# sair-lab/AirSLAM

Measured on AMD Instinct MI355X. Metric: stereo detect+match pairs/sec (2x PLNet @512x512 internal: points + lines, junctions on the left + LightGlue match), higher is better.
Workload: dtype fp16

## Files before the change

### airslam_amd/csrc/kernels_lgblockf.hip

```cpp
#include "common.h"
#include "kernels.h"
#ifdef LF_TIMING
__device__ unsigned long long lf_dbg[32];
#define LF_T(i) { const long long now_ = wall_clock64(); if (L.wave == 0 && L.lane == 0) atomicAdd(&lf_dbg[L.tb + i], (unsigned long long)(now_ - tp_)); tp_ = now_; }
extern "C" void airfe_dbg_lf(unsigned long long* out, int reset) {
  if (reset) { unsigned long long z[32] = {}; (void)hipMemcpyToSymbol(HIP_SYMBOL(lf_dbg), z, sizeof(z)); }
  else (void)hipMemcpyFromSymbol(out, HIP_SYMBOL(lf_dbg), 32 * sizeof(unsigned long long));
}
#else
#define LF_T(i)
#endif
#ifdef LF_TIMING2
__device__ unsigned long long lf2_dbg[16];
extern "C" void airfe_dbg_lf2(unsigned long long* out, int reset) {
  if (reset) { unsigned long long z[16] = {}; (void)hipMemcpyToSymbol(HIP_SYMBOL(lf2_dbg), z, sizeof(z)); }
  else (void)hipMemcpyFromSymbol(out, HIP_SYMBOL(lf2_dbg), 16 * sizeof(unsigned long long));
}
#define LF2_NOW(v) { __builtin_amdgcn_sched_barrier(0); v = __builtin_readcyclecounter(); __builtin_amdgcn_sched_barrier(0); }
#endif

namespace airfe {

constexpr int LF_R0 = 0, LF_R1 = 65536, LF_ST = 131072;
constexpr int LF_LDS = LF_ST + 8 * 128 * 8;

#ifndef LF_FRAG
#define LF_FRAG 1
#endif
constexpr int LF_SS = LF_FRAG ? 2048 : SLAB_BYTES;
constexpr int lf_ts(int K) { return LF_FRAG ? (K / 64) * 2048 : 2048; }
constexpr int LF_TS256 = lf_ts(256), LF_TS512 = lf_ts(512);
__device__ __forceinline__ size_t lf_woff(int K, int cb, int t0) {
  return LF_FRAG ? (size_t)(cb * 4 + t0) * (K / 64) * 2048 : (size_t)cb * (K / 64) * SLAB_BYTES + (size_t)t0 * 2048;
}

__device__ __forceinline__ void lf_glds16(const void* gsrc, unsigned lds_off) {
  unsigned keep;
  asm volatile("s_mov_b32 %0, m0\n\ts_mov_b32 m0, %2\n\ts_nop 0\n\tglobal_load_lds_dwordx4 %1, off\n\ts_mov_b32 m0, %0"
               : "=&s"(keep)
               : "v"(gsrc), "s"(lds_off)
               : "memory");
}

#ifndef LF_GELU_ERFC
__device__ __forceinline__ f32x2 lf_gelu2(f32x2 y) {
  const f32x2 t = {__builtin_amdgcn_fmed3f(y.x, -4.5f, 4.5f), __builtin_amdgcn_fmed3f(y.y, -4.5f, 4.5f)};
  const f32x2 x = (t * t) * (2.0f / 20.25f) - 1.0f;
  f32x2 r = x * 0.0031705170404165983f - 0.009152771905064583f;
  r = r * x + 0.012448843568563461f;
  r = r * x - 0.016971856355667114f;
  r = r * x + 0.027542514726519585f;
  r = r * x - 0.040475402027368546f;
  r = r * x + 0.05482625961303711f;
  r = r * x - 0.07717858254909515f;
  r = r * x + 0.15690208971500397f;
  return y * (t * r + 0.5f);
}
__device__ __forceinline__ void lf_gelu2x4(f32x2 (&y)[4]) {
  f32x2 t[4], x[4], r[4];
#define LF_G4(expr) _Pragma("unroll") for (int k = 0; k < 4; ++k) { expr; } __builtin_amdgcn_sched_barrier(0);
  LF_G4((t[k] = f32x2{__builtin_amdgcn_fmed3f(y[k].x, -4.5f, 4.5f), __builtin_amdgcn_fmed3f(y[k].y, -4.5f, 4.5f)}))
  LF_G4(x[k] = t[k] * t[k])
  LF_G4(x[k] = x[k] * (2.0f / 20.25f) - 1.0f)
  LF_G4(r[k] = x[k] * 0.0031705170404165983f - 0.009152771905064583f)
  LF_G4(r[k] = r[k] * x[k] + 0.012448843568563461f)
  LF_G4(r[k] = r[k] * x[k] - 0.016971856355667114f)
  LF_G4(r[k] = r[k] * x[k] + 0.027542514726519585f)
  LF_G4(r[k] = r[k] * x[k] - 0.040475402027368546f)
  LF_G4(r[k] = r[k] * x[k] + 0.05482625961303711f)
  LF_G4(r[k] = r[k] * x[k] - 0.07717858254909515f)
  LF_G4(r[k] = r[k] * x[k] + 0.15690208971500397f)
  LF_G4(r[k] = t[k] * r[k] + 0.5f)
  LF_G4(y[k] = y[k] * r[k])
#undef LF_G4
}
#else
__device__ __forceinline__ f32x2 lf_gelu2(f32x2 y) {
  const f32x2 a = __builtin_elementwise_abs(y);
  f32x2 x = a * 0.70710678118654752f;
  x = __builtin_elementwise_min(x, f32x2{6.0f, 6.0f});
  const f32x2 u = x * (1.0f / 3.0f) - 1.0f;
  f32x2 r = u * 0.008399954997003078f - 0.02763195149600506f;
  r = r * u + 0.04838801920413971f;
  r = r * u - 0.08357185125350952f;
  r = r * u + 0.1567264348268509f;
  r = r * u - 0.28920042514801025f;
  r = r * u + 0.5534077286720276f;
  r = r * u - 1.3146467208862305f;
  r = r * u - 2.481963634490967f;
  const f32x2 p = (x * x) * -1.4426950408889634f + r;
  const f32x2 q = {__builtin_amdgcn_exp2f(p.x), __builtin_amdgcn_exp2f(p.y)};
  return __builtin_elementwise_max(y, f32x2{0.f, 0.f}) - (x * 0.70710678118654752f) * q;
}
__device__ __forceinline__ void lf_gelu2x4(f32x2 (&y)[4]) {
#pragma unroll
  for (int k = 0; k < 4; ++k) y[k] = lf_gelu2(y[k]);
}
#endif

__device__ __forceinline__ void lf_stage_rows(const uint16_t* src, int row0, int nmt, int region, int wave, int lane) {
  for (int i = 0; i < nmt; ++i) {
    const int inst = wave * nmt + i;
    const int r = inst * 2 + (lane >> 5), pp = lane & 31;
    lf_glds16(src + (size_t)(row0 + r) * 256 + ((pp ^ (r & 15)) << 3), (unsigned)(region + inst * 1024));
  }
}

template <class P>
__device__ __forceinline__ typename P::vec8 lf_ldg(const char* p) {
  return __builtin_bit_cast(typename P::vec8, *reinterpret_cast<const uint4*>(p));
}

template <class P, int NT, int TS>
__device__ __forceinline__ void lf_first(typename P::vec8 (&cur)[NT][2], const char* w0, const char* w1) {
#pragma unroll
  for (int t = 0; t < NT; ++t) {
    cur[t][0] = lf_ldg<P>(w0 + t * TS);
    cur[t][1] = lf_ldg<P>(w1 + t * TS);
  }
}

struct LfNoHook { __device__ __forceinline__ void operator()(int) const {} };

#ifndef LF_GELU_X4
#define LF_GELU_X4 1
#endif


template <class P, int NT, int NMT, int TS, int TSN, class Hook = LfNoHook, bool SWAP = false, bool TIMED = false>
__device__ __forceinline__ void lf_mma(f32x4 (&acc)[NT][NMT], typename P::vec8 (&cur)[NT][2], const char* w0, const char* w1, int nslab,
                                       const char* n0, const char* n1, const char* breg, int pitch, int l15, int g, Hook hook = Hook()) {
  const char* brow = breg + l15 * pitch;
  if constexpr (NMT <= 4) {
    typename P::vec8 ring[8][NT][2];
    auto fetch = [&](int k, typename P::vec8 (&dst)[NT][2]) {
      const char* p0 = k == nslab ? n0 : w0 + k * LF_SS;
      const char* p1 = k == nslab ? n1 : w1 + k * LF_SS;
      const int ts = k == nslab ? TSN : TS;
#pragma unroll
      for (int t = 0; t < NT; ++t) {
        dst[t][0] = lf_ldg<P>(p0 + t * ts);
        dst[t][1] = lf_ldg<P>(p1 + t * ts);
      }
    };
    constexpr int AHEAD = (NT == 4 ? 4 : 8) / (NMT > 2 ? 2 : 1);
#pragma unroll
    for (int d = 1; d <= AHEAD; ++d)
      if (d <= nslab) fetch(d, ring[d - 1]);
    __builtin_amdgcn_sched_barrier(0);
#pragma unroll
    for (int s = 0; s < 8; ++s) {
      if (s < nslab) {
        hook(s);
        __builtin_amdgcn_sched_barrier(0);
#pragma unroll
        for (int h = 0; h < 2; ++h) {
          const int boff = (((s * 8 + h * 4 + g) ^ l15) << 4);
          typename P::vec8 bf[NMT];
#pragma unroll
          for (int j = 0; j < NMT; ++j) bf[j] = lds_frag<P>(brow, boff + j * 16 * pitch);
#pragma unroll
          for (int t = 0; t < NT; ++t)
#pragma unroll
            for (int j = 0; j < NMT; ++j) {
              if constexpr (SWAP) acc[t][j] = P::mfma(bf[j], cur[t][h], acc[t][j]);
              else acc[t][j] = P::mfma(cur[t][h], bf[j], acc[t][j]);
            }
        }
#pragma unroll
        for (int t = 0; t < NT; ++t) {
          cur[t][0] = ring[s % AHEAD][t][0];
          cur[t][1] = ring[s % AHEAD][t][1];
        }
        if (s + 1 + AHEAD <= nslab) fetch(s + 1 + AHEAD, ring[s % AHEAD]);
        __builtin_amdgcn_sched_barrier(0);
      }
    }
    return;
  }
  typename P::vec8 nxt[NT][2];
#ifdef LF_NOLDS
  typename P::vec8 bf0[4];
#pragma unroll
  for (int j = 0; j < 4; ++j) bf0[j] = lds_frag<P>(brow, ((g ^ l15) << 4) + j * 16 * pitch);
#endif
#ifdef LF_TIMING2
  [[maybe_unused]] unsigned long long q0 = 0, q1 = 0, q2 = 0, q3 = 0, q4 = 0, q5 = 0, q6 = 0;
  [[maybe_unused]] unsigned long long a_pref = 0, a_vm = 0, a_rd = 0, a_lgkm = 0, a_mma = 0, a_mov = 0, a_trips = 0;
#endif
#pragma unroll 1
  for (int s = 0; s < nslab; ++s) {
#ifdef LF_TIMING2
    if constexpr (TIMED) LF2_NOW(q0)
#endif
    const bool last = s + 1 == nslab;
    const char* p0 = last ? n0 : w0 + (s + 1) * LF_SS;
    const char* p1 = last ? n1 : w1 + (s + 1) * LF_SS;
#ifdef LF_NOWEIGHTS
    if (true) {
      (void)p0; (void)p1;
#pragma unroll
      for (int t = 0; t < NT; ++t) {
        nxt[t][0] = cur[t][0];
        nxt[t][1] = cur[t][1];
      }
    } else
#endif
    if constexpr (TS == TSN) {
#pragma unroll
      for (int t = 0; t < NT; ++t) {
        nxt[t][0] = lf_ldg<P>(p0 + t * TS);
        nxt[t][1] = lf_ldg<P>(p1 + t * TS);
      }
    } else {
      const int ts = last ? TSN : TS;
#pragma unroll
      for (int t = 0; t < NT; ++t) {
        nxt[t][0] = lf_ldg<P>(p0 + t * ts);
        nxt[t][1] = lf_ldg<P>(p1 + t * ts);
      }
    }
    hook(s);
    __builtin_amdgcn_sched_barrier(0);
#ifdef LF_TIMING2
    if constexpr (TIMED) {
      LF2_NOW(q1)
      asm volatile("s_waitcnt vmcnt(%0)" ::"n"(2 * NT) : "memory");
      LF2_NOW(q2)
      a_pref += q1 - q0; a_vm += q2 - q1;
    }
#endif
#pragma unroll
    for (int h = 0; h < 2; ++h) {
      const int boff = (((s * 8 + h * 4 + g) ^ l15) << 4);
#pragma unroll
      for (int mb = 0; mb < NMT; mb += 4) {
#ifdef LF_TIMING2
        if constexpr (TIMED) LF2_NOW(q3)
#endif
        typename P::vec8 bf[4];
#ifdef LF_NOLDS
        (void)boff;
#pragma unroll
        for (int j = 0; j < 4; ++j) bf[j] = bf0[j];
#else
#pragma unroll
        for (int j = 0; j < 4; ++j)
          if (mb + j < NMT) bf[j] = lds_frag<P>(brow, boff + (mb + j) * 16 * pitch);
#endif
#ifdef LF_TIMING2
        if constexpr (TIMED) {
          LF2_NOW(q4)
          asm volatile("s_waitcnt lgkmcnt(0)" ::: "memory");
          LF2_NOW(q5)
        }
#endif
#pragma unroll
        for (int t = 0; t < NT; ++t)
#pragma unroll
          for (int j = 0; j < 4; ++j)
            if (mb + j < NMT) {
              if constexpr (SWAP) acc[t][mb + j] = P::mfma(bf[j], cur[t][h], acc[t][mb + j]);
              else acc[t][mb + j] = P::mfma(cur[t][h], bf[j], acc[t][mb + j]);
            }
#ifdef LF_TIMING2
        if constexpr (TIMED) {
          LF2_NOW(q6)
          a_rd += q4 - q3; a_lgkm += q5 - q4; a_mma += q6 - q5;
        }
#endif
      }
    }
#pragma unroll
    for (int t = 0; t < NT; ++t) {
      cur[t][0] = nxt[t][0];
      cur[t][1] = nxt[t][1];
    }
#ifdef LF_TIMING2
    if constexpr (TIMED) {
      LF2_NOW(q1)
      a_mov += q1 - q6; a_trips += 1;
    }
#endif
  }
#ifdef LF_TIMING2
  if constexpr (TIMED) {
    if ((threadIdx.x & 63) == 0) {
      atomicAdd(&lf2_dbg[0], a_pref); atomicAdd(&lf2_dbg[1], a_vm); atomicAdd(&lf2_dbg[2], a_rd); atomicAdd(&lf2_dbg[3], a_lgkm); atomicAdd(&lf2_dbg[4], a_mma);
      atomicAdd(&lf2_dbg[5], a_mov); atomicAdd(&lf2_dbg[6], a_trips); atomicAdd(&lf2_dbg[7], (unsigned long long)(2 * ((NMT + 3) / 4)) * a_trips);
      atomicAdd(&lf2_dbg[8], (unsigned long long)(2 * NT * NMT) * a_trips);
    }
  }
#endif
}

struct LfLane {
  int lane, wave, l15, g, wf, cb, tp, fo0, fo1;
#ifdef LF_TIMING
  int tb;
#endif
  const char *wob, *w1b, *w2b;
};

template <class P, int NMT, bool RELU, int FOLD, bool FOLDO>
__device__ __forceinline__ void lf_pass(const LgBlockFArgs& a, char* smem, const LfLane& L, int row0) {
  const int lane = L.lane, wave = L.wave, l15 = L.l15, g = L.g, wf = L.wf, cb = L.cb, tp = L.tp, fo0 = L.fo0, fo1 = L.fo1;
#ifdef LF_TIMING
  long long tp_ = wall_clock64();
  if (wave == 0 && lane == 0) atomicAdd(&lf_dbg[L.tb + 15], 1ull);
#endif
  typename P::vec8 c2[2][2], c4[4][2];
  [[maybe_unused]] f32x4 bo2[2];
  f32x4 b14[4];
  if constexpr (FOLDO) {
    lf_first<P, 4, LF_TS512>(c4, L.w1b + 4 * LF_SS + fo0, L.w1b + 4 * LF_SS + fo1);
  } else {
    lf_first<P, 2, LF_TS256>(c2, L.wob + fo0, L.wob + fo1);
#pragma unroll
    for (int u = 0; u < 2; ++u) bo2[u] = *reinterpret_cast<const f32x4*>(a.bo + cb * 64 + tp * 32 + g * 8 + u * 4);
  }
#pragma unroll
  for (int t = 0; t < 4; ++t) b14[t] = *reinterpret_cast<const f32x4*>(a.b1 + wf * 64 + (t >> 1) * 32 + g * 8 + (t & 1) * 4);
  asm volatile("s_waitcnt vmcnt(0)" ::: "memory");
  __syncthreads();
  LF_T(0)

  if constexpr (!FOLDO) {
    {
    f32x4 acc[2][NMT];
#pragma unroll
    for (int u = 0; u < 2; ++u)
#pragma unroll
      for (int m = 0; m < NMT; ++m) acc[u][m] = bo2[u];
    lf_mma<P, 2, NMT, LF_TS256, LF_TS256>(acc, c2, L.wob + fo0, L.wob + fo1, 4, L.wob + fo0, L.wob + fo1, smem + LF_R0, 512, l15, g);
    lf_first<P, 4, LF_TS512>(c4, L.w1b + 4 * LF_SS + fo0, L.w1b + 4 * LF_SS + fo1);
    const int piece = cb * 8 + tp * 4 + g;
#pragma unroll
    for (int m = 0; m < NMT; ++m) {
      float v[8];
#pragma unroll
      for (int e = 0; e < 4; ++e) {
        v[e] = acc[0][m][e];
        v[4 + e] = acc[1][m][e];
      }
      *reinterpret_cast<uint4*>(smem + LF_R1 + (m * 16 + l15) * 512 + ((piece ^ l15) << 4)) = pack8<P>(v);
    }
    }
    __syncthreads();
  }
  LF_T(1)

  f32x4 h[4][NMT];
#pragma unroll
  for (int t = 0; t < 4; ++t)
#pragma unroll
    for (int m = 0; m < NMT; ++m) h[t][m] = b14[t];
  if constexpr (FOLDO) {
    lf_mma<P, 4, NMT, LF_TS512, LF_TS512>(h, c4, L.w1b + 4 * LF_SS + fo0, L.w1b + 4 * LF_SS + fo1, 4, L.w1b + fo0, L.w1b + fo1, smem + LF_R1, 512, l15, g);
    LF_T(2)
    LF_T(3)
  } else {
    auto xhook = [&](int s) { if (s == 3) lf_stage_rows(a.xb, row0, NMT, LF_R0, wave, lane); };
    lf_mma<P, 4, NMT, LF_TS512, LF_TS512, decltype(xhook)>(h, c4, L.w1b + 4 * LF_SS + fo0, L.w1b + 4 * LF_SS + fo1, 4, L.w1b + fo0, L.w1b + fo1, smem + LF_R1, 512, l15, g,
                                                             xhook);
    LF_T(2)
    asm volatile("s_waitcnt vmcnt(0)" ::: "memory");
    __syncthreads();
    LF_T(3)
  }
#ifdef LF_TIMING2
  lf_mma<P, 4, NMT, LF_TS512, LF_TS512, LfNoHook, false, true>(h, c4, L.w1b + fo0, L.w1b + fo1, 4, L.w1b + fo0, L.w1b + fo1, smem + LF_R0, 512, l15, g);
#else
  lf_mma<P, 4, NMT, LF_TS512, LF_TS512>(h, c4, L.w1b + fo0, L.w1b + fo1, 4, L.w1b + fo0, L.w1b + fo1, smem + LF_R0, 512, l15, g);
#endif

  [[maybe_unused]] f32x4 gam[2][2], bet[2][2];
  if constexpr (!RELU) {
#pragma unroll
    for (int q = 0; q < 2; ++q)
#pragma unroll
      for (int u = 0; u < 2; ++u) {
        gam[q][u] = *reinterpret_cast<const f32x4*>(a.gamma + wf * 64 + q * 32 + g * 8 + u * 4);
        bet[q][u] = *reinterpret_cast<const f32x4*>(a.beta + wf * 64 + q * 32 + g * 8 + u * 4);
      }
  }
  if constexpr (!RELU) {
    float2* st = reinterpret_cast<float2*>(smem + LF_ST);
#pragma unroll
    for (int m = 0; m < NMT; ++m) {
      float s1 = 0.f, s2 = 0.f;
#pragma unroll
      for (int t = 0; t < 4; ++t)
#pragma unroll
        for (int e = 0; e < 4; ++e) s1 += h[t][m][e];
      s1 = rows_sum(s1);
      const float mw = s1 * (1.0f / 64.0f);
#pragma unroll
      for (int t = 0; t < 4; ++t)
#pragma unroll
        for (int e = 0; e < 4; ++e) {
          const float d = h[t][m][e] - mw;
          s2 = fmaf(d, d, s2);
        }
      s2 = rows_sum(s2);
      if (g == 0) st[wf * 128 + m * 16 + l15] = make_float2(s1, s2);
    }
  }
  LF_T(4)
  __syncthreads();
  LF_T(5)
  const int co = cb * 64 + tp * 32 + g * 8;
  float* xr0 = a.x32 + (size_t)(row0 + l15) * 256 + co;
  float4 r0[NMT], r1[NMT];
  constexpr bool EARLY_W2 = NMT < 8;
  if constexpr (EARLY_W2) lf_first<P, 2, LF_TS512>(c2, L.w2b + fo0, L.w2b + fo1);
  f32x4 b22[2];
#pragma unroll
  for (int u = 0; u < 2; ++u) b22[u] = *reinterpret_cast<const f32x4*>(a.b2 + co + u * 4);
  __builtin_amdgcn_sched_barrier(0);
  {
    const float2* st = reinterpret_cast<const float2*>(smem + LF_ST);
    [[maybe_unused]] float nmr[NMT], rstd[NMT];
#pragma unroll
    for (int m = 0; m < (RELU ? 0 : NMT); ++m) {
      float s1 = 0.f, s2 = 0.f;
#pragma unroll
      for (int w = 0; w < 8; ++w) s1 += st[w * 128 + m * 16 + l15].x;
      const float mean = s1 * (1.0f / 512.0f);
#pragma unroll
      for (int w = 0; w < 8; ++w) {
        const float2 p = st[w * 128 + m * 16 + l15];
        const float dm = p.x * (1.0f / 64.0f) - mean;
        s2 += fmaf(64.0f * dm, dm, p.y);
      }
      const float var = s2 * (1.0f / 512.0f);
      rstd[m] = 1.0f / sqrtf(var + 1e-5f);
      nmr[m] = -mean * rstd[m];
    }
#pragma unroll
    for (int q = 0; q < 2; ++q) {
      const int piece = wf * 8 + q * 4 + g;
      if constexpr (RELU) {
#pragma unroll
        for (int m = 0; m < NMT; ++m) {
          float v[8];
#pragma unroll
          for (int e = 0; e < 4; ++e) {
            v[e] = fmaxf(h[2 * q][m][e], 0.f);
            v[4 + e] = fmaxf(h[2 * q + 1][m][e], 0.f);
          }
          *reinterpret_cast<uint4*>(smem + (m * 16 + l15) * 1024 + ((piece ^ l15) << 4)) = pack8<P>(v);
        }
      } else {
      const f32x4 g0 = gam[q][0], g1 = gam[q][1], be0 = bet[q][0], be1 = bet[q][1];
#pragma unroll
      for (int m = 0; m < NMT; ++m) {
        const f32x2 rs = {rstd[m], rstd[m]}, nm = {nmr[m], nmr[m]};
        float v[8];
#if LF_GELU_X4
        f32x2 y[4];
#pragma unroll
        for (int e = 0; e < 4; e += 2) {
          y[e >> 1] = (f32x2{h[2 * q][m][e], h[2 * q][m][e + 1]} * rs + nm) * f32x2{g0[e], g0[e + 1]} + f32x2{be0[e], be0[e + 1]};
          y[2 + (e >> 1)] = (f32x2{h[2 * q + 1][m][e], h[2 * q + 1][m][e + 1]} * rs + nm) * f32x2{g1[e], g1[e + 1]} + f32x2{be1[e], be1[e + 1]};
        }
        lf_gelu2x4(y);
#pragma unroll
        for (int e = 0; e < 4; e += 2) {
          v[e] = y[e >> 1].x; v[e + 1] = y[e >> 1].y;
          v[4 + e] = y[2 + (e >> 1)].x; v[5 + e] = y[2 + (e >> 1)].y;
        }
#else
#pragma unroll
        for (int e = 0; e < 4; e += 2) {
          const f32x2 y0 = (f32x2{h[2 * q][m][e], h[2 * q][m][e + 1]} * rs + nm) * f32x2{g0[e], g0[e + 1]} + f32x2{be0[e], be0[e + 1]};
          const f32x2 y1 = (f32x2{h[2 * q + 1][m][e], h[2 * q + 1][m][e + 1]} * rs + nm) * f32x2{g1[e], g1[e + 1]} + f32x2{be1[e], be1[e + 1]};
          const f32x2 o0 = lf_gelu2(y0), o1 = lf_gelu2(y1);
          v[e] = o0.x; v[e + 1] = o0.y;
          v[4 + e] = o1.x; v[5 + e] = o1.y;
        }
#endif
        *reinterpret_cast<uint4*>(smem + (m * 16 + l15) * 1024 + ((piece ^ l15) << 4)) = pack8<P>(v);
      }
      }
      if (q == 0) {
#pragma unroll
        for (int m = 0; m < NMT; ++m) {
          r0[m] = *reinterpret_cast<const float4*>(xr0 + (size_t)m * 16 * 256);
          r1[m] = *reinterpret_cast<const float4*>(xr0 + (size_t)m * 16 * 256 + 4);
        }
        __builtin_amdgcn_sched_barrier(0);
      }
    }
  }
  if constexpr (!EARLY_W2) lf_first<P, 2, LF_TS512>(c2, L.w2b + fo0, L.w2b + fo1);
  LF_T(6)
  __syncthreads();
  LF_T(7)

  constexpr bool KEEP_X = FOLD != 0 && NMT < 8;
  [[maybe_unused]] uint4 xpk[KEEP_X ? NMT : 1];
  {
    f32x4 acc[2][NMT];
#pragma unroll
    for (int u = 0; u < 2; ++u)
#pragma unroll
      for (int m = 0; m < NMT; ++m) acc[u][m] = b22[u];
    const char* nq = FOLD ? reinterpret_cast<const char*>(a.nqk_w) + lf_woff(256, cb, 2 * tp) : L.w2b;
    lf_mma<P, 2, NMT, LF_TS512, (FOLD ? LF_TS256 : LF_TS512)>(acc, c2, L.w2b + fo0, L.w2b + fo1, 8, nq + fo0, nq + fo1, smem, 1024, l15, g);
#pragma unroll
    for (int m = 0; m < NMT; ++m) {
      const size_t row = (size_t)(row0 + m * 16 + l15);
      float* xr = xr0 + (size_t)m * 16 * 256;
      float v[8] = {acc[0][m][0] + r0[m].x, acc[0][m][1] + r0[m].y, acc[0][m][2] + r0[m].z, acc[0][m][3] + r0[m].w,
                    acc[1][m][0] + r1[m].x, acc[1][m][1] + r1[m].y, acc[1][m][2] + r1[m].z, acc[1][m][3] + r1[m].w};
      *reinterpret_cast<float4*>(xr) = make_float4(v[0], v[1], v[2], v[3]);
      *reinterpret_cast<float4*>(xr + 4) = make_float4(v[4], v[5], v[6], v[7]);
      const uint4 xp = pack8<P>(v);
      if constexpr (KEEP_X) xpk[m] = xp;
      *reinterpret_cast<uint4*>(a.xb + row * 256 + co) = xp;
    }
  }
  LF_T(8)
  if constexpr (FOLD != 0) {
    __syncthreads();
    {
      const int piece = cb * 8 + tp * 4 + g;
#pragma unroll
      for (int m = 0; m < NMT; ++m) {
        uint4 xp;
        if constexpr (KEEP_X) xp = xpk[m];
        else xp = *reinterpret_cast<const uint4*>(a.xb + (size_t)(row0 + m * 16 + l15) * 256 + co);
        *reinterpret_cast<uint4*>(smem + LF_R0 + (m * 16 + l15) * 512 + ((piece ^ l15) << 4)) = xp;
      }
    }
    __syncthreads();
    LF_T(9)
    const int H = a.H, Np = a.Np;
    constexpr int NQ = FOLD == 2 ? 2 : 1;
    const char* vbase = reinterpret_cast<const char*>(a.nv_w) + lf_woff(256, cb, 2 * tp);
#pragma unroll
    for (int qu = 0; qu < NQ; ++qu) {
      const int cbq = cb + 4 * qu;
      const char* wq = reinterpret_cast<const char*>(a.nqk_w) + lf_woff(256, cbq, 2 * tp);
      const char* nx = (qu + 1 < NQ) ? reinterpret_cast<const char*>(a.nqk_w) + lf_woff(256, cbq + 4, 2 * tp) : vbase;
      const int cq = cbq * 64 + tp * 32 + g * 8;
      f32x4 bq[2];
#pragma unroll
      for (int u = 0; u < 2; ++u) bq[u] = *reinterpret_cast<const f32x4*>(a.nqk_b + cq + u * 4);
      f32x4 acc[2][NMT];
#pragma unroll
      for (int u = 0; u < 2; ++u)
#pragma unroll
        for (int m = 0; m < NMT; ++m) acc[u][m] = f32x4{0.f, 0.f, 0.f, 0.f};
      lf_mma<P, 2, NMT, LF_TS256, LF_TS256>(acc, c2, wq + fo0, wq + fo1, 4, nx + fo0, nx + fo1, smem + LF_R0, 512, l15, g);
      const int sel = cq >> 8, hh = (cq & 255) >> 6, d = cq & 63;
      uint16_t* ob = sel ? a.k_out : a.q_out;
#pragma unroll
      for (int m = 0; m < NMT; ++m) {
        const int row = row0 + m * 16 + l15;
        float v[8];
#pragma unroll
        for (int e = 0; e < 4; ++e) {
          v[e] = acc[0][m][e] + bq[0][e];
          v[4 + e] = acc[1][m][e] + bq[1][e];
        }
        if constexpr (FOLD == 2) {
          const f32x4 cs = *reinterpret_cast<const f32x4*>(a.rot_cos + (size_t)row * 32 + tp * 16 + g * 4);
          const f32x4 sn = *reinterpret_cast<const f32x4*>(a.rot_sin + (size_t)row * 32 + tp * 16 + g * 4);
          rotate_pairs(v, cs, sn);
        }
        const int sq = row / Np, nn = row - sq * Np;
        *reinterpret_cast<uint4*>(ob + (((size_t)sq * H + hh) * Np + nn) * 64 + d) = pack8<P>(v);
      }
    }
    LF_T(10)
    {
      float bt[2];
#pragma unroll
      for (int u = 0; u < 2; ++u) bt[u] = a.nv_b[cb * 64 + slab_row_to_feature((2 * tp + u) * 16 + l15)];
      f32x4 acc[2][NMT];
#pragma unroll
      for (int u = 0; u < 2; ++u)
#pragma unroll
        for (int m = 0; m < NMT; ++m) acc[u][m] = f32x4{0.f, 0.f, 0.f, 0.f};
      lf_mma<P, 2, NMT, LF_TS256, LF_TS256, LfNoHook, true>(acc, c2, vbase + fo0, vbase + fo1, 4, vbase + fo0, vbase + fo1, smem + LF_R0, 512, l15, g);
#pragma unroll
      for (int u = 0; u < 2; ++u) {
        const int cv = cb * 64 + slab_row_to_feature((2 * tp + u) * 16 + l15);
        const int hh = cv >> 6, d = cv & 63;
#pragma unroll
        for (int m = 0; m < NMT; ++m) {
          const int rw = row0 + m * 16 + g * 4;
          const int sq = rw / Np, nn = rw - sq * Np;
          *reinterpret_cast<uint2*>(a.vt_out + (((size_t)sq * H + hh) * 64 + d) * Np + nn) =
                pack4<P>(acc[u][m][0] + bt[u], acc[u][m][1] + bt[u], acc[u][m][2] + bt[u], acc[u][m][3] + bt[u]);
        }
      }
    }
    LF_T(11)
  }
}

__device__ __forceinline__ void lf_lane_init(const LgBlockFArgs& a, LfLane& L) {
  const int tid = threadIdx.x;
  L.lane = tid & 63;
  L.wave = __builtin_amdgcn_readfirstlane(tid >> 6);
  L.l15 = L.lane & 15;
  L.g = L.lane >> 4;
  if (LF_FRAG) {
    L.fo0 = L.lane * 16;
    L.fo1 = L.lane * 16 + 1024;
  } else {
    const int sw = (L.l15 >> 1) & 7;
    L.fo0 = L.l15 * 128 + ((L.g ^ sw) << 4);
    L.fo1 = L.l15 * 128 + (((4 + L.g) ^ sw) << 4);
  }
  L.wf = (L.wave + (blockIdx.x >> 3)) & 7;
  L.cb = L.wf >> 1;
  L.tp = L.wf & 1;
  L.wob = reinterpret_cast<const char*>(a.wo) + lf_woff(256, L.cb, 2 * L.tp);
  L.w1b = reinterpret_cast<const char*>(a.w1) + lf_woff(512, L.wf, 0);
  L.w2b = reinterpret_cast<const char*>(a.w2) + lf_woff(512, L.cb, 2 * L.tp);
}

template <class P, int NMT, bool RELU, int FOLD, bool FOLDO>
__global__ __launch_bounds__(512, 1) void lg_blockf_kernel(LgBlockFArgs a) {
  extern __shared__ __attribute__((aligned(16))) char smem[];
  LfLane L;
  lf_lane_init(a, L);
  const int row0 = blockIdx.x * (16 * NMT);
  lf_stage_rows(a.attn, row0, NMT, FOLDO ? LF_R1 : LF_R0, L.wave, L.lane);
  if constexpr (FOLDO) lf_stage_rows(a.xb, row0, NMT, LF_R0, L.wave, L.lane);
#ifdef LF_TIMING
  L.tb = 0;
#endif
  lf_pass<P, NMT, RELU, FOLD, FOLDO>(a, smem, L, row0);
#ifdef LF_TWICE
  __syncthreads();
  L.tb = 16;
  lf_stage_rows(a.attn, row0, NMT, FOLDO ? LF_R1 : LF_R0, L.wave, L.lane);
  if constexpr (FOLDO) lf_stage_rows(a.xb, row0, NMT, LF_R0, L.wave, L.lane);
  lf_pass<P, NMT, RELU, FOLD, FOLDO>(a, smem, L, row0);
#endif
}

template <class P, bool RELU, int FOLD>
__global__ __launch_bounds__(512, 1) void lg_blockf_mixed_kernel(LgBlockFArgs a, int n7) {
  extern __shared__ __attribute__((aligned(16))) char smem[];
  LfLane L;
  lf_lane_init(a, L);
#ifdef LF_TIMING
  L.tb = 0;
#endif
  if ((int)blockIdx.x < n7) {
    const int row0 = blockIdx.x * 112;
    lf_stage_rows(a.attn, row0, 7, LF_R1, L.wave, L.lane);
    lf_stage_rows(a.xb, row0, 7, LF_R0, L.wave, L.lane);
    lf_pass<P, 7, RELU, FOLD, true>(a, smem, L, row0);
  } else {
    const int row0 = n7 * 112 + ((int)blockIdx.x - n7) * 96;
    lf_stage_rows(a.attn, row0, 6, LF_R1, L.wave, L.lane);
    lf_stage_rows(a.xb, row0, 6, LF_R0, L.wave, L.lane);
    lf_pass<P, 6, RELU, FOLD, true>(a, smem, L, row0);
  }
}

template <class P, bool RELU, int FOLD>
static bool launch_mixed(const LgBlockFArgs& a, hipStream_t st) {
  const int tiles = (a.M + 15) / 16, W = a.n_cu;
  if (!a.mixed || a.wo || W <= 0 || tiles <= 7 * W || tiles > 13 * W) return false;
  const int n7 = W, n6 = (tiles - 7 * W + 5) / 6;
  static PerDeviceOnce attr_once;
  auto kfn = lg_blockf_mixed_kernel<P, RELU, FOLD>;
  if (auto once_token = attr_once.first()) {
    (void)hipFuncSetAttribute(reinterpret_cast<const void*>(kfn), hipFuncAttributeMaxDynamicSharedMemorySize, LF_LDS);
  }
  hipLaunchKernelGGL(kfn, dim3((unsigned)(n7 + n6)), dim3(512), LF_LDS, st, a, n7);
  return true;
}

template <class P, int NMT, bool RELU, int FOLD, bool FOLDO>
static void launch_fo(const LgBlockFArgs& a, hipStream_t st) {
  static PerDeviceOnce attr_once;
  auto kfn = lg_blockf_kernel<P, NMT, RELU, FOLD, FOLDO>;
  if (auto once_token = attr_once.first()) {
    (void)hipFuncSetAttribute(reinterpret_cast<const void*>(kfn), hipFuncAttributeMaxDynamicSharedMemorySize, LF_LDS);
  }
  hipLaunchKernelGGL(kfn, dim3((unsigned)((a.M + 16 * NMT - 1) / (16 * NMT))), dim3(512), LF_LDS, st, a);
}

template <class P, int NMT, bool RELU, int FOLD = 0>
static void launch_f(const LgBlockFArgs& a, hipStream_t st) {
  if (a.wo) launch_fo<P, NMT, RELU, FOLD, false>(a, st);
  else launch_fo<P, NMT, RELU, FOLD, true>(a, st);
}

template <class P, bool RELU, int FOLD>
static void launch_nmt(const LgBlockFArgs& a, hipStream_t st) {
  switch (a.tokens_per_wg) {
    case 32: launch_f<P, 2, RELU, FOLD>(a, st); break;
    case 64: launch_f<P, 4, RELU, FOLD>(a, st); break;
    case 112: if (!launch_mixed<P, RELU, FOLD>(a, st)) launch_f<P, 7, RELU, FOLD>(a, st); break;
    default: launch_f<P, 8, RELU, FOLD>(a, st); break;
  }
}

bool lg_blockf_frag_weights() { return LF_FRAG != 0; }

void launch_lg_blockf(int prec, const LgBlockFArgs& a, hipStream_t st) {
  if (a.relu) {
    if (prec == 1) launch_nmt<PF16, true, 0>(a, st); else launch_nmt<PBF16, true, 0>(a, st);
    return;
  }
  if (a.nqk_w) {
    if (a.nqk_n == 512) {
      if (prec == 1) launch_nmt<PF16, false, 2>(a, st); else launch_nmt<PBF16, false, 2>(a, st);
    } else {
      if (prec == 1) launch_nmt<PF16, false, 1>(a, st); else launch_nmt<PBF16, false, 1>(a, st);
    }
    return;
  }
  if (prec == 1) launch_nmt<PF16, false, 0>(a, st); else launch_nmt<PBF16, false, 0>(a, st);
}

}
```

Measured before the change: 8092.

## Merge folded Q/K/V projection GEMMs into one wider MMA pass with LDS-staged rotary tables

In the folded LightGlue block kernel, the separate per-unit Q/K (and V) projection passes are merged into a single 4-tile MMA loop that streams two weight units at once, using a per-tile offset and a per-tile operand-swap threshold. Rotary cos/sin tables are prefetched early and staged in LDS so the rotation epilogue reads shared memory instead of global. Output stores use incremental address arithmetic instead of per-row division. This is meant to cut repeated B-fragment LDS reads, loop overhead, and global latency in the epilogue, at the cost of higher register pressure from the doubled accumulators.

Measured after the change: 8072, median of 3. About the same (-0.3%).

```diff
diff --git a/airslam_amd/csrc/kernels_lgblockf.hip b/airslam_amd/csrc/kernels_lgblockf.hip
--- a/airslam_amd/csrc/kernels_lgblockf.hip
+++ b/airslam_amd/csrc/kernels_lgblockf.hip
@@ -1,11 +1,11 @@
 #include "common.h"
 #include "kernels.h"
 #ifdef LF_TIMING
-__device__ unsigned long long lf_dbg[32];
+__device__ unsigned long long lf_dbg[96];
 #define LF_T(i) { const long long now_ = wall_clock64(); if (L.wave == 0 && L.lane == 0) atomicAdd(&lf_dbg[L.tb + i], (unsigned long long)(now_ - tp_)); tp_ = now_; }
 extern "C" void airfe_dbg_lf(unsigned long long* out, int reset) {
-  if (reset) { unsigned long long z[32] = {}; (void)hipMemcpyToSymbol(HIP_SYMBOL(lf_dbg), z, sizeof(z)); }
-  else (void)hipMemcpyFromSymbol(out, HIP_SYMBOL(lf_dbg), 32 * sizeof(unsigned long long));
+  if (reset) { unsigned long long z[96] = {}; (void)hipMemcpyToSymbol(HIP_SYMBOL(lf_dbg), z, sizeof(z)); }
+  else (void)hipMemcpyFromSymbol(out, HIP_SYMBOL(lf_dbg), 96 * sizeof(unsigned long long));
 }
 #else
 #define LF_T(i)
@@ -127,20 +127,23 @@
 #endif
 
 
-template <class P, int NT, int NMT, int TS, int TSN, class Hook = LfNoHook, bool SWAP = false, bool TIMED = false>
+template <class P, int NT, int NMT, int TS, int TSN, class Hook = LfNoHook, int SW = NT, bool TIMED = false>
 __device__ __forceinline__ void lf_mma(f32x4 (&acc)[NT][NMT], typename P::vec8 (&cur)[NT][2], const char* w0, const char* w1, int nslab,
-                                       const char* n0, const char* n1, const char* breg, int pitch, int l15, int g, Hook hook = Hook()) {
+                                       const char* n0, const char* n1, const char* breg, int pitch, int l15, int g, Hook hook = Hook(),
+                                       long xo = 0, long xon = 0) {
   const char* brow = breg + l15 * pitch;
+  auto toff = [](int t, int ts, long x) { return (long)t * ts + (t >= NT / 2 ? x : 0l); };
   if constexpr (NMT <= 4) {
     typename P::vec8 ring[8][NT][2];
     auto fetch = [&](int k, typename P::vec8 (&dst)[NT][2]) {
       const char* p0 = k == nslab ? n0 : w0 + k * LF_SS;
       const char* p1 = k == nslab ? n1 : w1 + k * LF_SS;
       const int ts = k == nslab ? TSN : TS;
+      const long x = k == nslab ? xon : xo;
 #pragma unroll
       for (int t = 0; t < NT; ++t) {
-        dst[t][0] = lf_ldg<P>(p0 + t * ts);
-        dst[t][1] = lf_ldg<P>(p1 + t * ts);
+        dst[t][0] = lf_ldg<P>(p0 + toff(t, ts, x));
+        dst[t][1] = lf_ldg<P>(p1 + toff(t, ts, x));
       }
     };
     constexpr int AHEAD = (NT == 4 ? 4 : 8) / (NMT > 2 ? 2 : 1);
@@ -163,7 +166,7 @@
           for (int t = 0; t < NT; ++t)
 #pragma unroll
             for (int j = 0; j < NMT; ++j) {
-              if constexpr (SWAP) acc[t][j] = P::mfma(bf[j], cur[t][h], acc[t][j]);
+              if (t >= SW) acc[t][j] = P::mfma(bf[j], cur[t][h], acc[t][j]);
               else acc[t][j] = P::mfma(cur[t][h], bf[j], acc[t][j]);
             }
         }
@@ -206,18 +209,19 @@
       }
     } else
 #endif
+    const long x = last ? xon : xo;
     if constexpr (TS == TSN) {
 #pragma unroll
       for (int t = 0; t < NT; ++t) {
-        nxt[t][0] = lf_ldg<P>(p0 + t * TS);
-        nxt[t][1] = lf_ldg<P>(p1 + t * TS);
+        nxt[t][0] = lf_ldg<P>(p0 + toff(t, TS, x));
+        nxt[t][1] = lf_ldg<P>(p1 + toff(t, TS, x));
       }
     } else {
       const int ts = last ? TSN : TS;
 #pragma unroll
       for (int t = 0; t < NT; ++t) {
-        nxt[t][0] = lf_ldg<P>(p0 + t * ts);
-        nxt[t][1] = lf_ldg<P>(p1 + t * ts);
+        nxt[t][0] = lf_ldg<P>(p0 + toff(t, ts, x));
+        nxt[t][1] = lf_ldg<P>(p1 + toff(t, ts, x));
       }
     }
     hook(s);
@@ -260,7 +264,7 @@
 #pragma unroll
           for (int j = 0; j < 4; ++j)
             if (mb + j < NMT) {
-              if constexpr (SWAP) acc[t][mb + j] = P::mfma(bf[j], cur[t][h], acc[t][mb + j]);
+              if (t >= SW) acc[t][mb + j] = P::mfma(bf[j], cur[t][h], acc[t][mb + j]);
               else acc[t][mb + j] = P::mfma(cur[t][h], bf[j], acc[t][mb + j]);
             }
 #ifdef LF_TIMING2
@@ -292,6 +296,19 @@
     }
   }
 #endif
+}
+
+#ifndef LF_FOLD_MERGE
+#define LF_FOLD_MERGE 3
+#endif
+#ifndef LF_ROT_LDS
+#define LF_ROT_LDS 1
+#endif
+
+template <int FOLD>
+__device__ __forceinline__ const char* lf_fold_unit2(const LgBlockFArgs& a, int cb, int tp) {
+  if constexpr (FOLD == 2) return reinterpret_cast<const char*>(a.nqk_w) + lf_woff(256, cb + 4, 2 * tp);
+  else return reinterpret_cast<const char*>(a.nv_w) + lf_woff(256, cb, 2 * tp);
 }
 
 struct LfLane {
@@ -369,7 +386,7 @@
     LF_T(3)
   }
 #ifdef LF_TIMING2
-  lf_mma<P, 4, NMT, LF_TS512, LF_TS512, LfNoHook, false, true>(h, c4, L.w1b + fo0, L.w1b + fo1, 4, L.w1b + fo0, L.w1b + fo1, smem + LF_R0, 512, l15, g);
+  lf_mma<P, 4, NMT, LF_TS512, LF_TS512, LfNoHook, 4, true>(h, c4, L.w1b + fo0, L.w1b + fo1, 4, L.w1b + fo0, L.w1b + fo1, smem + LF_R0, 512, l15, g);
 #else
   lf_mma<P, 4, NMT, LF_TS512, LF_TS512>(h, c4, L.w1b + fo0, L.w1b + fo1, 4, L.w1b + fo0, L.w1b + fo1, smem + LF_R0, 512, l15, g);
 #endif
@@ -499,6 +516,21 @@
   LF_T(7)
 
   constexpr bool KEEP_X = FOLD != 0 && NMT < 8;
+  constexpr bool ROTL = LF_ROT_LDS != 0 && FOLD == 2 && ((LF_FOLD_MERGE >> 1) & 1) != 0 && NMT < 8;
+  constexpr int NRC = (4 * NMT + 7) / 8;
+  [[maybe_unused]] f32x4 rotp[ROTL ? NRC : 1];
+  if constexpr (ROTL) {
+#pragma unroll
+    for (int i = 0; i < NRC; ++i) {
+      const int c = wave + 8 * i;
+      if (c < 4 * NMT) {
+        const float* tb = c < 2 * NMT ? a.rot_cos : a.rot_sin;
+        rotp[i] = *reinterpret_cast<const f32x4*>(tb + (size_t)row0 * 32 + (c < 2 * NMT ? c : c - 2 * NMT) * 256 + lane * 4);
+      }
+    }
+    __builtin_amdgcn_sched_barrier(0);
+  }
+  constexpr bool MERGE = FOLD != 0 && ((LF_FOLD_MERGE >> (FOLD ? FOLD - 1 : 0)) & 1) != 0 && NMT < 8;
   [[maybe_unused]] uint4 xpk[KEEP_X ? NMT : 1];
   {
     f32x4 acc[2][NMT];
@@ -508,6 +540,14 @@
       for (int m = 0; m < NMT; ++m) acc[u][m] = b22[u];
     const char* nq = FOLD ? reinterpret_cast<const char*>(a.nqk_w) + lf_woff(256, cb, 2 * tp) : L.w2b;
     lf_mma<P, 2, NMT, LF_TS512, (FOLD ? LF_TS256 : LF_TS512)>(acc, c2, L.w2b + fo0, L.w2b + fo1, 8, nq + fo0, nq + fo1, smem, 1024, l15, g);
+    if constexpr (MERGE) {
+      const char* u2 = lf_fold_unit2<FOLD>(a, cb, tp);
+#pragma unroll
+      for (int t = 0; t < 2; ++t) {
+        c4[2 + t][0] = lf_ldg<P>(u2 + fo0 + t * LF_TS256);
+        c4[2 + t][1] = lf_ldg<P>(u2 + fo1 + t * LF_TS256);
+      }
+    }
 #pragma unroll
     for (int m = 0; m < NMT; ++m) {
       const size_t row = (size_t)(row0 + m * 16 + l15);
@@ -534,11 +574,148 @@
         *reinterpret_cast<uint4*>(smem + LF_R0 + (m * 16 + l15) * 512 + ((piece ^ l15) << 4)) = xp;
       }
     }
+    if constexpr (ROTL) {
+#pragma unroll
+      for (int i = 0; i < NRC; ++i) {
+        const int c = wave + 8 * i;
+        if (c < 4 * NMT) *reinterpret_cast<f32x4*>(smem + LF_R1 + (c < 2 * NMT ? c * 1024 : 16384 + (c - 2 * NMT) * 1024) + lane * 16) = rotp[i];
+      }
+    }
     __syncthreads();
     LF_T(9)
     const int H = a.H, Np = a.Np;
     constexpr int NQ = FOLD == 2 ? 2 : 1;
     const char* vbase = reinterpret_cast<const char*>(a.nv_w) + lf_woff(256, cb, 2 * tp);
+    if constexpr (MERGE) {
+      const char* wq = reinterpret_cast<const char*>(a.nqk_w) + lf_woff(256, cb, 2 * tp);
+      const long xo = (lf_fold_unit2<FOLD>(a, cb, tp) - wq) - 2 * LF_TS256;
+      f32x4 bq[NQ][2];
+      float bt[2];
+#pragma unroll
+      for (int qu = 0; qu < NQ; ++qu)
+#pragma unroll
+        for (int u = 0; u < 2; ++u) bq[qu][u] = *reinterpret_cast<const f32x4*>(a.nqk_b + (cb + 4 * qu) * 64 + tp * 32 + g * 8 + u * 4);
+#pragma unroll
+      for (int u = 0; u < 2; ++u) bt[u] = a.nv_b[cb * 64 + slab_row_to_feature((2 * tp + u) * 16 + l15)];
+#pragma unroll
+      for (int t = 0; t < 2; ++t) {
+        c4[t][0] = c2[t][0];
+        c4[t][1] = c2[t][1];
+      }
+      f32x4 acc[4][NMT];
+#pragma unroll
+      for (int t = 0; t < 4; ++t)
+#pragma unroll
+        for (int m = 0; m < NMT; ++m) acc[t][m] = f32x4{0.f, 0.f, 0.f, 0.f};
+      if constexpr (FOLD == 2)
+        lf_mma<P, 4, NMT, LF_TS256, LF_TS256>(acc, c4, wq + fo0, wq + fo1, 4, vbase + fo0, vbase + fo1, smem + LF_R0, 512, l15, g, LfNoHook(), xo, -2l * LF_TS256);
+      else
+        lf_mma<P, 4, NMT, LF_TS256, LF_TS256, LfNoHook, 2>(acc, c4, wq + fo0, wq + fo1, 4, wq + fo0, wq + fo1, smem + LF_R0, 512, l15, g, LfNoHook(), xo, xo);
+      LF_T(12)
+      uint4 pk[NQ][NMT];
+      [[maybe_unused]] f32x4 cs[FOLD == 2 ? NMT : 1], sn[FOLD == 2 ? NMT : 1];
+      if constexpr (FOLD == 2) {
+#pragma unroll
+        for (int m = 0; m < NMT; ++m) {
+          if constexpr (ROTL) {
+            const char* rl = smem + LF_R1 + (m * 16 + l15) * 128 + tp * 64 + g * 16;
+            cs[m] = *reinterpret_cast<const f32x4*>(rl);
+            sn[m] = *reinterpret_cast<const f32x4*>(rl + 16384);
+          } else {
+            const size_t ro = (size_t)(row0 + m * 16 + l15) * 32 + tp * 16 + g * 4;
+            cs[m] = *reinterpret_cast<const f32x4*>(a.rot_cos + ro);
+            sn[m] = *reinterpret_cast<const f32x4*>(a.rot_sin + ro);
+          }
+        }
+        __builtin_amdgcn_sched_barrier(0);
+      }
+#pragma unroll
+      for (int m = 0; m < NMT; ++m)
+#pragma unroll
+        for (int qu = 0; qu < NQ; ++qu) {
+          float v[8];
+#pragma unroll
+          for (int e = 0; e < 4; ++e) {
+            v[e] = acc[2 * qu][m][e] + bq[qu][0][e];
+            v[4 + e] = acc[2 * qu + 1][m][e] + bq[qu][1][e];
+          }
+          if constexpr (FOLD == 2) rotate_pairs(v, cs[m], sn[m]);
+          pk[qu][m] = pack8<P>(v);
+        }
+      LF_T(10)
+      f32x4 vacc[2][NMT];
+      if constexpr (FOLD == 2) {
+#pragma unroll
+        for (int u = 0; u < 2; ++u) {
+          c2[u][0] = c4[u][0];
+          c2[u][1] = c4[u][1];
+#pragma unroll
+          for (int m = 0; m < NMT; ++m) vacc[u][m] = f32x4{0.f, 0.f, 0.f, 0.f};
+        }
+        lf_mma<P, 2, NMT, LF_TS256, LF_TS256, LfNoHook, 0>(vacc, c2, vbase + fo0, vbase + fo1, 4, vbase + fo0, vbase + fo1, smem + LF_R0, 512, l15, g);
+      } else {
+#pragma unroll
+        for (int u = 0; u < 2; ++u)
+#pragma unroll
+          for (int m = 0; m < NMT; ++m) vacc[u][m] = acc[2 + u][m];
+      }
+      LF_T(13)
+      auto stores = [&](auto fastc) {
+        constexpr bool FAST = decltype(fastc)::value;
+        {
+          size_t cu[2];
+#pragma unroll
+          for (int u = 0; u < 2; ++u) cu[u] = (size_t)(cb * 64 + slab_row_to_feature((2 * tp + u) * 16 + l15)) * Np;
+          const size_t seq = (size_t)H * 64 * Np;
+          int sq = (row0 + g * 4) / Np, nn = (row0 + g * 4) - sq * Np;
+          size_t vo = (size_t)sq * seq + nn;
+#pragma unroll
+          for (int m = 0; m < NMT; ++m) {
+#pragma unroll
+            for (int u = 0; u < 2; ++u)
+              *reinterpret_cast<uint2*>(a.vt_out + vo + cu[u]) =
+                    pack4<P>(vacc[u][m][0] + bt[u], vacc[u][m][1] + bt[u], vacc[u][m][2] + bt[u], vacc[u][m][3] + bt[u]);
+            if constexpr (FAST) {
+              nn += 16; vo += 16;
+              if (nn >= Np) { nn -= Np; vo += seq - Np; }
+            } else {
+              const int rw = row0 + (m + 1) * 16 + g * 4;
+              sq = rw / Np; nn = rw - sq * Np;
+              vo = (size_t)sq * seq + nn;
+            }
+          }
+        }
+        {
+          size_t cq[NQ];
+          uint16_t* ob[NQ];
+#pragma unroll
+          for (int qu = 0; qu < NQ; ++qu) {
+            const int c = (cb + 4 * qu) * 64 + tp * 32 + g * 8;
+            ob[qu] = (c >> 8) ? a.k_out : a.q_out;
+            cq[qu] = (size_t)((c & 255) >> 6) * Np * 64 + (c & 63);
+          }
+          const size_t seq = (size_t)H * Np * 64;
+          int sq = (row0 + l15) / Np, nn = (row0 + l15) - sq * Np;
+          size_t qo = (size_t)sq * seq + (size_t)nn * 64;
+#pragma unroll
+          for (int m = 0; m < NMT; ++m) {
+#pragma unroll
+            for (int qu = 0; qu < NQ; ++qu) *reinterpret_cast<uint4*>(ob[qu] + qo + cq[qu]) = pk[qu][m];
+            if constexpr (FAST) {
+              nn += 16; qo += 16 * 64;
+              if (nn >= Np) { nn -= Np; qo += seq - (size_t)Np * 64; }
+            } else {
+              const int row = row0 + (m + 1) * 16 + l15;
+              sq = row / Np; nn = row - sq * Np;
+              qo = (size_t)sq * seq + (size_t)nn * 64;
+            }
+          }
+        }
+      };
+      if (Np >= 16) stores(std::true_type{});
+      else stores(std::false_type{});
+      LF_T(11)
+    } else {
 #pragma unroll
     for (int qu = 0; qu < NQ; ++qu) {
       const int cbq = cb + 4 * qu;
@@ -554,6 +731,7 @@
 #pragma unroll
         for (int m = 0; m < NMT; ++m) acc[u][m] = f32x4{0.f, 0.f, 0.f, 0.f};
       lf_mma<P, 2, NMT, LF_TS256, LF_TS256>(acc, c2, wq + fo0, wq + fo1, 4, nx + fo0, nx + fo1, smem + LF_R0, 512, l15, g);
+      LF_T(12)
       const int sel = cq >> 8, hh = (cq & 255) >> 6, d = cq & 63;
       uint16_t* ob = sel ? a.k_out : a.q_out;
 #pragma unroll
@@ -573,8 +751,8 @@
         const int sq = row / Np, nn = row - sq * Np;
         *reinterpret_cast<uint4*>(ob + (((size_t)sq * H + hh) * Np + nn) * 64 + d) = pack8<P>(v);
       }
-    }
-    LF_T(10)
+      LF_T(10)
+    }
     {
       float bt[2];
 #pragma unroll
@@ -584,7 +762,8 @@
       for (int u = 0; u < 2; ++u)
 #pragma unroll
         for (int m = 0; m < NMT; ++m) acc[u][m] = f32x4{0.f, 0.f, 0.f, 0.f};
-      lf_mma<P, 2, NMT, LF_TS256, LF_TS256, LfNoHook, true>(acc, c2, vbase + fo0, vbase + fo1, 4, vbase + fo0, vbase + fo1, smem + LF_R0, 512, l15, g);
+      lf_mma<P, 2, NMT, LF_TS256, LF_TS256, LfNoHook, 0>(acc, c2, vbase + fo0, vbase + fo1, 4, vbase + fo0, vbase + fo1, smem + LF_R0, 512, l15, g);
+      LF_T(13)
 #pragma unroll
       for (int u = 0; u < 2; ++u) {
         const int cv = cb * 64 + slab_row_to_feature((2 * tp + u) * 16 + l15);
@@ -599,6 +778,7 @@
       }
     }
     LF_T(11)
+    }
   }
 }
 
@@ -633,12 +813,12 @@
   lf_stage_rows(a.attn, row0, NMT, FOLDO ? LF_R1 : LF_R0, L.wave, L.lane);
   if constexpr (FOLDO) lf_stage_rows(a.xb, row0, NMT, LF_R0, L.wave, L.lane);
 #ifdef LF_TIMING
-  L.tb = 0;
+  L.tb = 32 * FOLD;
 #endif
   lf_pass<P, NMT, RELU, FOLD, FOLDO>(a, smem, L, row0);
 #ifdef LF_TWICE
   __syncthreads();
-  L.tb = 16;
+  L.tb = 32 * FOLD + 16;
   lf_stage_rows(a.attn, row0, NMT, FOLDO ? LF_R1 : LF_R0, L.wave, L.lane);
   if constexpr (FOLDO) lf_stage_rows(a.xb, row0, NMT, LF_R0, L.wave, L.lane);
   lf_pass<P, NMT, RELU, FOLD, FOLDO>(a, smem, L, row0);
@@ -651,7 +831,7 @@
   LfLane L;
   lf_lane_init(a, L);
 #ifdef LF_TIMING
-  L.tb = 0;
+  L.tb = 32 * FOLD + ((int)blockIdx.x < n7 ? 0 : 16);
 #endif
   if ((int)blockIdx.x < n7) {
     const int row0 = blockIdx.x * 112;
```
